# ZechengLi19/CIM

Hardware: AMD Instinct MI355X
Metric: images/sec training step (ResNet-50 VOC, ~1k proposals/img) at 1/2/4/8 GPU (higher is better)
Workload: dtype fp32

## Files before the change

cim_amd/csrc/losses.hip:

```cpp
#include "common.h"
#include "wave_block.h"
#include "../../include/cim_hip.h"
#include <limits.h>

namespace {

constexpr int NT = 1024;
constexpr float LO = 1e-6f, HI = 1.0f - 1e-6f;
#ifndef CIM_LOSS_CLOCKS
#define CIM_LOSS_CLOCKS 0
#endif
#if CIM_LOSS_CLOCKS
__device__ unsigned long long g_loss_clk[8][16];
#define LCLK(JOB, I) do { if (threadIdx.x == 0 && (JOB) < 8) g_loss_clk[JOB][I] = wall_clock64(); } while (0)
#else
#define LCLK(JOB, I) do { } while (0)
#endif

__device__ __forceinline__ float clampf(float x) { return fminf(fmaxf(x, LO), HI); }
__device__ __forceinline__ float inrange(float x) { return (x >= LO && x <= HI) ? 1.0f : 0.0f; }

__device__ float block_sum(float v, float* red) {
#pragma unroll
    for (int o = 32; o > 0; o >>= 1) v += __shfl_xor(v, o);
    const int wave = threadIdx.x >> 6, lane = threadIdx.x & 63;
    __syncthreads();
    if (lane == 0) red[wave] = v;
    __syncthreads();
    float s = 0.0f;
    for (int w = 0; w < NT / 64; ++w) s += red[w];
    return s;
}

__device__ void block_sum4(float& v0, float& v1, float& v2, float& v3, float* buf) {
#pragma unroll
    for (int o = 32; o > 0; o >>= 1) {
// ... 386 lines not shown
                    if (row_cluster[n] != k) continue;
                    const float x = a.pc[(size_t)n * LD + c], p = clampf(x);
                    const float t = (row_col[n] == c) ? 1.0f : 0.0f;
                    s += -(t * logf(p) + (1.0f - t) * logf(1.0f - p));
                    g[(size_t)n * C1 + c] = scale * (-(t / p - (1.0f - t) / (1.0f - p))) / (float)C1 * inrange(x);
                }
    #pragma unroll
                for (int o = 32; o > 0; o >>= 1) s += __shfl_xor(s, o);
                if (lane == 0) acc += s / (float)C1;
            } else {
                float s = 0.0f;
                int any = 0;
                for (int n = lane; n < N; n += 64) {
                    if (row_cluster[n] != k) continue;
                    s += a.pc[(size_t)n * LD + c];
                    any |= (row_col[n] == c);
                }
    #pragma unroll
                for (int o = 32; o > 0; o >>= 1) { s += __shfl_xor(s, o); any |= __shfl_xor(any, o); }
                const float v = s / nk, p = clampf(v), t = any ? 1.0f : 0.0f;
                if (lane == 0) acc += nk * (-(t * logf(p) + (1.0f - t) * logf(1.0f - p))) / (float)C1;
                const float dv = scale * (-(t / p - (1.0f - t) / (1.0f - p))) / (float)C1 * inrange(v);
                for (int n = lane; n < N; n += 64)
                    if (row_cluster[n] == k) g[(size_t)n * C1 + c] = dv;
            }
        }
    }
    LCLK(a.R + 1, 3);
    acc = block_sum(acc, red);
    float* out = a.part + 4 * (a.R + 1);
    if (tid == 0) { out[0] = 0.f; out[1] = scale * acc; out[2] = 0.f; out[3] = 0.f; }
}

__global__ __launch_bounds__(NT) void losses_kernel(const cim_loss_args a) {
    extern __shared__ __attribute__((aligned(16))) unsigned char smem[];
    float* red = reinterpret_cast<float*>(smem);
    int* hot = reinterpret_cast<int*>(smem + 64);
    float* grp_scratch = reinterpret_cast<float*>(smem + 64 + 8 * (size_t)a.N);
    const int job = blockIdx.x;
    LCLK(job, 0);
    if (job < a.R) refine_job(a, job, red, hot, grp_scratch);
    else if (job == a.R) mil_job(a, red, grp_scratch);
    else pcl_job(a, red, smem + 64, grp_scratch);
    LCLK(job, 7);
}

}

#if CIM_LOSS_CLOCKS
extern "C" int cim_debug_loss_clocks(unsigned long long* host_out) {
    return hipMemcpyFromSymbol(host_out, HIP_SYMBOL(g_loss_clk), sizeof(g_loss_clk)) == hipSuccess ? 0 : 1;
}
#endif

extern "C" int cim_losses_fwd(const cim_loss_args* args, void* stream) {
    CIM_CHECK_ARG(args != nullptr);
    const cim_loss_args& a = *args;
    CIM_CHECK_ARG(a.N > 0 && a.N <= 15000 && a.C1 > 1 && a.C1 <= 32767 && a.R >= 0 && a.R <= 3 && (a.ld == 0 || a.ld >= a.C1));
    CIM_CHECK_ARG(a.pc && a.pd && a.labels && a.part && a.grad && a.mat && (a.R == 0 || a.layer_valid));
    for (int i = 0; i < a.R; ++i)
        CIM_CHECK_ARG(a.rc[i] && a.ri[i] && a.pseudo_labels[i] && a.pseudo_iou_f16[i] && a.loss_weights[i]);
    const int lg = a.C1 <= 32 ? 32 : a.C1 <= 64 ? 64 : a.C1 <= 128 ? 128 : a.C1 <= 256 ? 256 : 1024;
    const size_t lds = 64 + 8 * (size_t)a.N + (lg <= 256 ? 16 * (size_t)(NT / lg) * a.C1 + 16 : 0) + 256;
    if (lds > 64 * 1024)
        CIM_CHECK_HIP(hipFuncSetAttribute(reinterpret_cast<const void*>(losses_kernel),
                                          hipFuncAttributeMaxDynamicSharedMemorySize, (int)lds));
    hipLaunchKernelGGL(losses_kernel, dim3(a.R + 2), dim3(NT), lds, cim::as_stream(stream), a);
    CIM_CHECK_LAUNCH();
    return 0;
}

namespace {

__global__ __launch_bounds__(256) void head_colstat_kernel(const float* __restrict__ x, int N, int C1, int ld, int off,
                                                           float* __restrict__ stat) {
    __shared__ float red[4];
    const int c = blockIdx.x, tid = threadIdx.x;
    float m = -INFINITY;
    for (int n = tid; n < N; n += 256) m = fmaxf(m, x[(size_t)n * ld + off + c]);
#pragma unroll
    for (int o = 32; o > 0; o >>= 1) m = fmaxf(m, __shfl_xor(m, o));
    if ((tid & 63) == 0) red[tid >> 6] = m;
    __syncthreads();
    m = fmaxf(fmaxf(red[0], red[1]), fmaxf(red[2], red[3]));
    __syncthreads();
    float s = 0.0f;
    for (int n = tid; n < N; n += 256) s += expf(x[(size_t)n * ld + off + c] - m);
#pragma unroll
    for (int o = 32; o > 0; o >>= 1) s += __shfl_xor(s, o);
    if ((tid & 63) == 0) red[tid >> 6] = s;
    __syncthreads();
    if (tid == 0) {
        stat[c] = m;
        stat[C1 + c] = red[0] + red[1] + red[2] + red[3];
    }
}

__global__ __launch_bounds__(256) void head_act_fwd_kernel(const float* __restrict__ x, float* __restrict__ y, int N, int C1,
                                                           int R, const float* __restrict__ stat) {
    const int row = blockIdx.x * 4 + (threadIdx.x >> 6), lane = threadIdx.x & 63;
    if (row >= N) return;
    const int ld = (2 + 2 * R) * C1;
// ... 27 lines not shown
    for (int n = tid; n < N; n += 256) s += y[(size_t)n * ld + off + c] * dy[(size_t)n * ld + off + c];
#pragma unroll
    for (int o = 32; o > 0; o >>= 1) s += __shfl_xor(s, o);
    if ((tid & 63) == 0) red[tid >> 6] = s;
    __syncthreads();
    if (tid == 0) dot[c] = red[0] + red[1] + red[2] + red[3];
}

__global__ __launch_bounds__(256) void head_act_bwd_kernel(const float* __restrict__ y, const float* __restrict__ dy,
                                                           float* __restrict__ dx, int N, int C1, int R,
                                                           const float* __restrict__ dot) {
    const int row = blockIdx.x * 4 + (threadIdx.x >> 6), lane = threadIdx.x & 63;
    if (row >= N) return;
    const int ld = (2 + 2 * R) * C1;
    const float* yr = y + (size_t)row * ld;
    const float* gr = dy + (size_t)row * ld;
    float* dr = dx + (size_t)row * ld;
    for (int b = 0; b < 2 + 2 * R; ++b) {
        const int off = b * C1;
        if (b == 1) {
            for (int c = lane; c < C1; c += 64) dr[off + c] = yr[off + c] * (gr[off + c] - dot[c]);
        } else if (b < 2 + R) {
            float s = 0.0f;
            for (int c = lane; c < C1; c += 64) s += yr[off + c] * gr[off + c];
#pragma unroll
            for (int o = 32; o > 0; o >>= 1) s += __shfl_xor(s, o);
            for (int c = lane; c < C1; c += 64) dr[off + c] = yr[off + c] * (gr[off + c] - s);
        } else {
            for (int c = lane; c < C1; c += 64) dr[off + c] = gr[off + c] * yr[off + c] * (1.0f - yr[off + c]);
        }
    }
}

struct LossGrads { const float* p[6]; };
__global__ __launch_bounds__(256) void loss_grad_combine_kernel(const float* __restrict__ G, const LossGrads g,
                                                                float* __restrict__ out, int N, int C1, int R) {
    const size_t plane = (size_t)N * C1;
    const size_t i = (size_t)blockIdx.x * 256 + threadIdx.x;
    if (i >= plane) return;
    const int n = (int)(i / C1), c = (int)(i - (size_t)n * C1);
    float v[6];
#pragma unroll
    for (int k = 0; k < 6; ++k) v[k] = g.p[k] ? g.p[k][0] : 0.0f;
    const float g_bag = v[0] + v[5], g_pcl = v[1] + v[5], g_cls = v[2] + v[5], g_iou = v[3] + 3.0f * (v[4] + v[5]);
    float* o = out + (size_t)n * (2 + 2 * R) * C1 + c;
    o[0] = g_bag * G[i] + g_pcl * G[plane + i];
    o[C1] = g_bag * G[2 * plane + i];
    for (int r = 0; r < R; ++r) {
        const float* Gr = G + (size_t)(3 + 4 * r) * plane + i;
        o[(2 + r) * C1] = g_cls * Gr[0] + g_bag * Gr[plane];
        o[(2 + R + r) * C1] = g_iou * Gr[2 * plane] + g_bag * Gr[3 * plane];
    }
}

__global__ void loss_finish_kernel(const float* __restrict__ part, int rows, float* __restrict__ out) {
#pragma clang fp contract(off)
    const int k = threadIdx.x;
    float s = 0.0f;
    if (k < 4)
        for (int r = 0; r < rows; ++r) s += part[r * 4 + k];
    const float bag = __shfl(s, 0), pcl = __shfl(s, 1), cls = __shfl(s, 2), iou = __shfl(s, 3);
    if (k < 4) out[k] = s;
    if (k == 4) out[4] = 3.0f * iou;
    if (k == 5) out[5] = ((bag + pcl) + cls) + 3.0f * iou;
}

}

extern "C" int cim_loss_finish(const float* part, int rows, float* out, void* stream) {
    CIM_CHECK_ARG(part && out && rows > 0);
    hipLaunchKernelGGL(loss_finish_kernel, dim3(1), dim3(64), 0, cim::as_stream(stream), part, rows, out);
    CIM_CHECK_LAUNCH();
    return 0;
}

extern "C" int cim_loss_grad_combine(const float* G, const float* g_bag, const float* g_pcl, const float* g_cls, const float* g_iou,
                                     const float* g_iou3, const float* g_total, float* out, int N, int C1, int R, void* stream) {
    CIM_CHECK_ARG(G && out && N > 0 && C1 > 0 && R >= 0 && R <= 3);
    const LossGrads g{{g_bag, g_pcl, g_cls, g_iou, g_iou3, g_total}};
    const size_t n = (size_t)N * C1;
    hipLaunchKernelGGL(loss_grad_combine_kernel, dim3((unsigned)((n + 255) / 256)), dim3(256), 0, cim::as_stream(stream), G, g, out, N, C1, R);
    CIM_CHECK_LAUNCH();
    return 0;
}

extern "C" int cim_head_act_fwd(const float* logits, float* scores, float* colstat, int N, int C1, int R, void* stream) {
    CIM_CHECK_ARG(logits && scores && colstat && N > 0 && C1 > 0 && R >= 0 && R <= 8);
    const int ld = (2 + 2 * R) * C1;
    hipStream_t st = cim::as_stream(stream);
    hipLaunchKernelGGL(head_colstat_kernel, dim3(C1), dim3(256), 0, st, logits, N, C1, ld, C1, colstat);
    hipLaunchKernelGGL(head_act_fwd_kernel, dim3((N + 3) / 4), dim3(256), 0, st, logits, scores, N, C1, R, colstat);
    CIM_CHECK_LAUNCH();
    return 0;
}

extern "C" int cim_head_act_bwd(const float* scores, const float* grad_scores, float* grad_logits, float* coldot, int N,
                                int C1, int R, void* stream) {
    CIM_CHECK_ARG(scores && grad_scores && grad_logits && coldot && N > 0 && C1 > 0 && R >= 0 && R <= 8);
    const int ld = (2 + 2 * R) * C1;
    hipStream_t st = cim::as_stream(stream);
    hipLaunchKernelGGL(head_coldot_kernel, dim3(C1), dim3(256), 0, st, scores, grad_scores, N, C1, ld, C1, coldot);
    hipLaunchKernelGGL(head_act_bwd_kernel, dim3((N + 3) / 4), dim3(256), 0, st, scores, grad_scores, grad_logits, N, C1, R,
                       coldot);
    CIM_CHECK_LAUNCH();
    return 0;
}
```

cim_amd/modeling/heads.py:

```python
import ctypes
import os
import warnings

import numpy as np
import torch
import torch.nn as nn
import torch.nn.functional as F

from .. import _lib
from ..utils import engine

_EPS = 1e-6


def _clamp(x):
    return x.clamp(_EPS, 1 - _EPS)


def mil_loss(cls_score, labels, loss_weight=None):
    s = _clamp(cls_score)
    t = labels.clamp(0, 1)
    loss = -(t * torch.log(s)) - (1 - t) * torch.log(1 - s)
    if loss_weight is not None:
        loss = loss * loss_weight
    return loss.mean()


def _pad_bg(labels):
    return torch.cat((labels.new_ones(labels.shape[0], 1), labels), dim=1)


def mil_bag_loss(predict_cls, predict_det, labels):
    pred = _clamp((predict_cls * predict_det).sum(dim=0, keepdim=True))
    target = _pad_bg(labels) if pred.shape[-1] - 1 == labels.shape[-1] else labels
    return -(target * torch.log(pred) + (1 - target) * torch.log(1 - pred)).mean()
# ... 60 lines not shown
def PCL_loss(predict_cls, mat, labels):
    ids = torch.unique(mat)
    ids = ids[ids != 0]
    if ids.numel() == 0:
        return 12 * predict_cls.new_zeros(())
    col0 = torch.unique(mat[:, 0])
    col0 = col0[col0 != 0]
    assert col0.numel() <= 1
    eq = mat.unsqueeze(0) == ids.view(-1, 1, 1)
    rows = eq.any(dim=2).to(predict_cls.dtype)
    cols = eq.any(dim=1).to(predict_cls.dtype)
    n_k = rows.sum(dim=1)
    is_bg = (ids == col0[0]) if col0.numel() == 1 else torch.zeros_like(ids, dtype=torch.bool)
    p = _clamp(predict_cls)
    mean_vec = _clamp((rows @ predict_cls) / n_k.clamp(min=1).unsqueeze(1))
    fg_term = (-(cols * torch.log(mean_vec)) - (1 - cols) * torch.log(1 - mean_vec)).mean(dim=1)
    gt = (mat != 0).to(predict_cls.dtype)
    bce_rows = (-(gt * torch.log(p)) - (1 - gt) * torch.log(1 - p)).mean(dim=1)
    bg_term = (rows * bce_rows.unsqueeze(0)).sum(dim=1) / n_k.clamp(min=1)
    term = torch.where(is_bg, bg_term, fg_term) * n_k
    return 12 * (term.sum() / (1e-6 + n_k.sum()))


_LossArgs = _lib.STRUCTS["cim_loss_args"]


STATUS_BITS = {1: "a class produced more than K pseudo ground truths (internal)",
               2: "the pre-drawn uniforms were exhausted (internal)",
               4: "`mat` has rows with several non-zero entries: the fused PCL loss handles the reference's "
                  "one-cluster-per-row format (tools/pre/AGPL_label_assign.py:137-185) - set CIM_PCL_GENERAL=1 for the "
                  "general ATen formulation",
               8: "several distinct cluster ids in column 0 of `mat` (heads.py:20 asserts at most one)",
               16: "more PRM clusters in `mat` than the fused PCL loss supports - set CIM_PCL_GENERAL=1"}


class FusedLossFunction(torch.autograd.Function):

    @staticmethod
    def forward(ctx, meta, pc, pd, *scores):
        R = meta["R"]
        fused = meta.get("fused", False)
        dev = pc.device
        if fused:
            all_scores = pc.contiguous()
            N, C1 = all_scores.shape[0], all_scores.shape[1] // (2 + 2 * R)
            base, blk = all_scores.data_ptr(), 4 * C1
            ptrs = [base + h * blk for h in range(2 + 2 * R)]
            ld = (2 + 2 * R) * C1
        else:
            rc, ri = scores[:R], scores[R:2 * R]
            N, C1 = pc.shape
            pc, pd = pc.contiguous(), pd.contiguous()
            rc = [t.contiguous() for t in rc]
            ri = [t.contiguous() for t in ri]
            ptrs = [pc.data_ptr(), pd.data_ptr()] + [t.data_ptr() for t in rc] + [t.data_ptr() for t in ri]
            ld = 0
        part = torch.empty((R + 2, 4), dtype=torch.float32, device=dev)
        grad = torch.empty((3 + 4 * R, N, C1), dtype=torch.float32, device=dev)
        a = _LossArgs()
        a.pc, a.pd, a.ld = ptrs[0], ptrs[1], ld
        keep = []
        for i in range(R):
            a.rc[i], a.ri[i] = ptrs[2 + i], ptrs[2 + R + i]
            y, t16, w = (x.contiguous() for x in meta["pseudo"][i])
            assert t16.dtype == torch.float16 and y.dtype == torch.float32 and w.dtype == torch.float32
            keep += [y, t16, w]
            a.pseudo_labels[i], a.pseudo_iou_f16[i], a.loss_weights[i] = y.data_ptr(), t16.data_ptr(), w.data_ptr()
            a.weight_scale[i] = float(meta["scales"][i])
        labels = meta["labels"].reshape(-1).to(torch.float32).contiguous()
        mat = meta["mat"].to(torch.float32).contiguous()
        assert tuple(mat.shape) == (N, C1), "mat must be [N, C+1]"
        valid, status = meta["valid"], meta["status"]
        a.labels, a.mat = labels.data_ptr(), mat.data_ptr()
        a.layer_valid, a.status = _lib.ptr(valid), status.data_ptr()
        a.N, a.C1, a.R = N, C1, R
        a.part, a.grad = part.data_ptr(), grad.data_ptr()
        _lib.call("cim_losses_fwd", ctypes.byref(a), _lib.stream_ptr())
        ctx.R, ctx.fused, ctx.dims = R, fused, (N, C1)
        ctx.save_for_backward(grad)
        ctx.set_materialize_grads(False)
        out = torch.empty(6, dtype=torch.float32, device=dev)
        _lib.call("cim_loss_finish", part.data_ptr(), R + 2, out.data_ptr(), _lib.stream_ptr())
        return tuple(out.unbind(0))

    @staticmethod
    def backward(ctx, *g):
        (G,) = ctx.saved_tensors
        R = ctx.R
        if _rng.pending is not None and not LAZY_SETTLE:
            engine.queue_callback(settle_rng)
        _order_callers_stream_after_backward(G.device)
        if ctx.fused:
            N, C1 = ctx.dims
            out = torch.empty((N, (2 + 2 * R) * C1), dtype=torch.float32, device=G.device)
            g = [None if t is None else t.contiguous() for t in g]
            _lib.call("cim_loss_grad_combine", G.data_ptr(), *[_lib.ptr(t) for t in g], out.data_ptr(), N, C1, R, _lib.stream_ptr())
            return None, out, None
        zero = G.new_zeros(())
        v = [zero if t is None else t for t in g]
        g_bag, g_pcl, g_cls, g_iou = v[0] + v[5], v[1] + v[5], v[2] + v[5], v[3] + 3 * (v[4] + v[5])
        d_pc = g_bag * G[0] + g_pcl * G[1]
        d_pd = g_bag * G[2]
        d_rc = [g_cls * G[3 + 4 * i] + g_bag * G[4 + 4 * i] for i in range(R)]
        d_ri = [g_iou * G[5 + 4 * i] + g_bag * G[6 + 4 * i] for i in range(R)]
        return (None, d_pc, d_pd, *d_rc, *d_ri)


def _order_callers_stream_after_backward(dev):
    from ..ops import gemm as _g
    if not (engine.HAS_ENGINE_CALLBACK and _g.HIGH_PRIO and dev.type == "cuda"):
        return

    def order():
        cur = torch.cuda.current_stream(dev)
        hp = _g.main_stream_high_priority(dev)
# ... 22 lines not shown
def fused_losses(predict_cls, predict_det, ref_cls_score, ref_iou_score, labels, pseudo, scales, mat,
                 valid=None, status=None, with_total=False):
    R = len(ref_cls_score)
    dev = predict_cls.device
    pseudo = list(pseudo)
    if valid is None or any(ps is None for ps in pseudo):
        host_valid = torch.tensor([0 if ps is None else 1 for ps in pseudo], dtype=torch.int32)
        valid = host_valid.to(dev) if valid is None else valid * host_valid.to(dev)
        some = next((ps for ps in pseudo if ps is not None), None)
        if some is None:
            n, c1 = predict_cls.shape
            some = (predict_cls.new_zeros((n, c1)), torch.zeros(n, dtype=torch.float16, device=dev), predict_cls.new_zeros(n))
        pseudo = [some if ps is None else ps for ps in pseudo]
    own_status = status is None
    if own_status:
        status = torch.zeros(1, dtype=torch.int32, device=dev)
    meta = dict(R=R, pseudo=pseudo, scales=list(scales), labels=labels, mat=mat, valid=valid, status=status)
    base = _fused_base(predict_cls, predict_det, ref_cls_score, ref_iou_score)
    if base is not None:
        meta["fused"] = True
        out = FusedLossFunction.apply(meta, base, None)
    else:
        out = FusedLossFunction.apply(meta, predict_cls, predict_det, *ref_cls_score, *ref_iou_score)
    if own_status:
        check_status(int(status.item()))
    return tuple(out) if with_total else (out[0], out[1], out[2], out[3])


def check_status(word):
    if word:
        raise _lib.CimHipError("; ".join(msg for bit, msg in STATUS_BITS.items() if word & bit))


class cls_iou_model(nn.Module):

    def __init__(self, dim_in, dim_out, refine_times, class_agnostic=False):
        super().__init__()
        self.classifier = nn.Linear(dim_in, dim_out)
        self.detector = nn.Linear(dim_in, dim_out)
        self.refine_cls = nn.ModuleList([nn.Linear(dim_in, dim_out) for _ in range(refine_times)])
        self.refine_iou = nn.ModuleList([nn.Linear(dim_in, dim_out) for _ in range(refine_times)])

    def detectron_weight_mapping(self):
        return {name: name for name, _ in self.named_parameters()}, []

    def forward(self, seg_feature):
        if seg_feature.dim() == 4:
            seg_feature = seg_feature.squeeze(3).squeeze(2)
        layers = [self.classifier, self.detector] + list(self.refine_cls) + list(self.refine_iou)
        r = len(self.refine_cls)
        c1 = self.classifier.out_features
        if seg_feature.is_cuda and seg_feature.dtype == torch.float32:
            scores = HeadsFunction.apply(seg_feature, c1, r, *[l.weight for l in layers], *[l.bias for l in layers]).split(c1, dim=1)
        else:
            w = torch.cat([l.weight for l in layers], dim=0)
            b = torch.cat([l.bias for l in layers], dim=0)
            logits = F.linear(seg_feature, w, b)
            lg = logits.split(c1, dim=1)
            scores = ([F.softmax(lg[0], dim=-1), F.softmax(lg[1], dim=0)] + [F.softmax(l, dim=-1) for l in lg[2:2 + r]]
                      + [torch.sigmoid(l) for l in lg[2 + r:2 + 2 * r]])
        return scores[0], scores[1], list(scores[2:2 + r]), list(scores[2 + r:2 + 2 * r])


class HeadActFunction(torch.autograd.Function):

    @staticmethod
    def forward(ctx, logits, c1, r):
        logits = logits.contiguous()
        n = logits.shape[0]
        scores = torch.empty_like(logits)
        stat = torch.empty(2 * c1, dtype=torch.float32, device=logits.device)
        _lib.call("cim_head_act_fwd", logits.data_ptr(), scores.data_ptr(), stat.data_ptr(), n, c1, r, _lib.stream_ptr())
        ctx.save_for_backward(scores)
        ctx.dims = (n, c1, r)
        return scores

    @staticmethod
    def backward(ctx, g):
        (scores,) = ctx.saved_tensors
        n, c1, r = ctx.dims
        g = g.contiguous()
        dx = torch.empty_like(scores)
        dot = torch.empty(c1, dtype=torch.float32, device=scores.device)
        _lib.call("cim_head_act_bwd", scores.data_ptr(), g.data_ptr(), dx.data_ptr(), dot.data_ptr(), n, c1, r,
                  _lib.stream_ptr())
        return dx, None, None


def _small_gemm(a, b, c, m, n, k, lda, ldb, ldc, a_mcontig, b_kcontig):
    splits = _lib.call("cim_gemm_small_splits", m, n, k)
    ws = torch.empty(splits * m * n, dtype=torch.float32, device=c.device) if splits > 1 else None
    _lib.call("cim_gemm_small_f32", a.data_ptr(), b.data_ptr(), c.data_ptr(), m, n, k, lda, ldb, ldc, int(a_mcontig), int(b_kcontig),
              None, None, None, None, None, 0.0, None, 0, splits, _lib.ptr(ws), _lib.stream_ptr())


class HeadsFunction(torch.autograd.Function):

    @staticmethod
    def forward(ctx, x, c1, r, *wb):
        nh = 2 + 2 * r
        ws_, bs_ = wb[:nh], wb[nh:]
        x = x.contiguous()
        n, k = x.shape
        wcat = torch.cat([w.detach() for w in ws_], dim=0)
        bcat = torch.cat([b.detach() for b in bs_], dim=0)
        m = nh * c1
        logits = torch.empty((n, m), dtype=torch.float32, device=x.device)
        splits = _lib.call("cim_gemm_small_splits", n, m, k)
        wsp = torch.empty(splits * n * m, dtype=torch.float32, device=x.device) if splits > 1 else None
        _lib.call("cim_linear_bias_f32", x.data_ptr(), wcat.data_ptr(), bcat.data_ptr(), logits.data_ptr(), n, m, k, splits,
                  _lib.ptr(wsp), _lib.stream_ptr())
        scores = torch.empty_like(logits)
        stat = torch.empty(2 * c1, dtype=torch.float32, device=x.device)
        _lib.call("cim_head_act_fwd", logits.data_ptr(), scores.data_ptr(), stat.data_ptr(), n, c1, r, _lib.stream_ptr())
        ctx.save_for_backward(x, wcat, scores)
        ctx.dims = (n, k, c1, r)
        return scores

    @staticmethod
    def backward(ctx, g):
        x, wcat, scores = ctx.saved_tensors
        n, k, c1, r = ctx.dims
        nh = 2 + 2 * r
        m = nh * c1
        g = g.contiguous()
        dl = torch.empty_like(scores)
        dot = torch.empty(c1, dtype=torch.float32, device=scores.device)
        _lib.call("cim_head_act_bwd", scores.data_ptr(), g.data_ptr(), dl.data_ptr(), dot.data_ptr(), n, c1, r, _lib.stream_ptr())
        dx = dw = db = None
        if ctx.needs_input_grad[0]:
            dx = torch.empty((n, k), dtype=torch.float32, device=x.device)
            _small_gemm(dl, wcat, dx, n, k, m, m, k, k, False, False)
        if any(ctx.needs_input_grad[3:3 + nh]):
            dw = torch.empty((m, k), dtype=torch.float32, device=x.device)
            _small_gemm(dl, x, dw, m, k, n, m, k, k, True, False)
        if any(ctx.needs_input_grad[3 + nh:]):
            db = dl.sum(dim=0)
        gw = [dw[h * c1:(h + 1) * c1] if dw is not None and ctx.needs_input_grad[3 + h] else None for h in range(nh)]
        gb = [db[h * c1:(h + 1) * c1] if db is not None and ctx.needs_input_grad[3 + nh + h] else None for h in range(nh)]
        return (dx, None, None, *gw, *gb)


_MiningLayer = _lib.STRUCTS["cim_mining_layer"]
_MiningArgs = _lib.STRUCTS["cim_mining_args"]
MAX_LAYERS = _lib.CONSTANTS["CIM_MAX_LAYERS"]


class _RngLedger:

    def __init__(self):
        self.pending = None
        self.snapshot = None

    def draw(self, n):
        self.settle()
        before = np.random.get_state()
        u = np.random.random_sample(n)
        self.snapshot = (before, np.random.get_state())
        return u

    def commit(self, meta_dev):
        host = torch.empty(meta_dev.numel(), dtype=torch.int32, pin_memory=True)
        host.copy_(meta_dev, non_blocking=True)
        ev = torch.cuda.Event()
        ev.record()
        self.pending = (self.snapshot, host, ev)
        self.snapshot = None
        return host, ev

    def settle(self):
        if self.pending is None:
            return
        snapshot, host, ev = self.pending
# ... 285 lines not shown
```

cim_amd/modeling/model_builder.py:

```python
import importlib
import logging
import os
import pickle
from functools import wraps

import torch
import torch.nn as nn

from ..core.config import cfg
from ..ops import RoIAlign, RoIPool
from ..ops import gemm as _gemm_ops
from . import heads

logger = logging.getLogger(__name__)


def get_func(func_name):
    if func_name == "":
        return None
    try:
        parts = func_name.split(".")
        if len(parts) == 1:
            return globals()[parts[0]]
        module = importlib.import_module(__package__ + "." + ".".join(parts[:-1]))
# ... 81 lines not shown

    def state_dict(self, *args, **kwargs):
        _gemm_ops.wait_pending_updates()
        return super().state_dict(*args, **kwargs)

    def forward(self, data, rois, masks, labels, gtrois=None, mat=None, path=None, index=None,
                iou_map=None, asy_iou_map=None):
        if not (self.training and _gemm_ops.HIGH_PRIO and torch.is_tensor(data) and data.is_cuda) or torch.cuda.is_current_stream_capturing():
            return self._forward_impl(data, rois, masks, labels, gtrois, mat, path, index, iou_map, asy_iou_map)
        dev = data.device
        cur, hp = torch.cuda.current_stream(dev), _gemm_ops.main_stream_high_priority(dev)
        if cur == hp:
            return self._forward_impl(data, rois, masks, labels, gtrois, mat, path, index, iou_map, asy_iou_map)
        hp.wait_stream(cur)
        for t in (data, rois, masks, labels, gtrois, mat, index, iou_map, asy_iou_map):
            if torch.is_tensor(t) and t.is_cuda:
                t.record_stream(hp)
        with torch.cuda.stream(hp):
            out = self._forward_impl(data, rois, masks, labels, gtrois, mat, path, index, iou_map, asy_iou_map)
        cur.wait_stream(hp)
        out["blob_conv"].record_stream(cur)
        for v in out.get("losses", {}).values():
            v.record_stream(cur)
        return out

    def _forward_impl(self, data, rois, masks, labels, gtrois=None, mat=None, path=None, index=None,
                      iou_map=None, asy_iou_map=None):
        with torch.set_grad_enabled(self.training):
            im_data = data
            if self.training:
                _gemm_ops.join_side(discard=True)
                if hasattr(self.Box_Head, "prefetch"):
                    self.Box_Head.prefetch()
                dev, dt = im_data.device, im_data.dtype
                rois = rois.squeeze(dim=0).to(device=dev, dtype=dt)
                masks = masks.squeeze(dim=0).to(device=dev, dtype=dt)
                labels = labels.squeeze(dim=0).to(device=dev, dtype=dt)
                mat = mat.squeeze(dim=0).to(device=dev, dtype=dt)
                if index is not None:
                    index = index.squeeze(dim=0).to(device=dev).long()
            return_dict = {}
            prep = None
            if self.training and asy_iou_map is not None and asy_iou_map.is_cuda:
                prep = heads.prepare_containment(self.CIM_layer_list, asy_iou_map, self.using_CIM)
            blob_conv = self._conv_body(im_data)
            return_dict["blob_conv"] = blob_conv
            seg_x = self.Box_Head(blob_conv, rois, masks.detach())
            predict_cls, predict_det, ref_cls_score, ref_iou_score = self.cls_iou_model(seg_x)

            if not self.training:
                return testing_function(predict_cls, predict_det, ref_cls_score, ref_iou_score, return_dict)

            if iou_map is None or asy_iou_map is None:
                stem = os.path.splitext(os.path.split(path)[1])[0]
                iou_map = _load_map(cfg.iou_dir, stem, "iou_map", labels.device, index)
                asy_iou_map = _load_map(cfg.asy_iou_dir, stem, "asy_iou_map", labels.device, index)

            scores = [(predict_cls, predict_det) if i == 0 else (ref_cls_score[i - 1], ref_iou_score[i - 1])
                      for i in range(len(self.CIM_layer_list))]
            mined = self.__dict__.get("_fixed_mining")
            if mined is None:
                mined = heads.mine_step(self.CIM_layer_list, scores, labels, iou_map, asy_iou_map, self.using_CIM, prep=prep)
            scales = [3 if i == 0 else 1 for i in range(len(self.CIM_layer_list))]
            if cfg.REFINE_TIMES <= 3 and not PCL_GENERAL:
                bag, pcl, cls_l, _, iou3, total = heads.fused_losses(predict_cls, predict_det, ref_cls_score, ref_iou_score,
                                                                     labels, mined.pseudo, scales, mat, valid=mined.valid,
# ... 79 lines not shown
```

cim_amd/nn/parallel/data_parallel.py:

```python
import os
import contextlib

import torch
import torch.distributed as dist

from ...ops.gemm import join_side as _join_side, gradient_is_deferred as _gradient_is_deferred
from ...ops import gemm as _gemm_ops
from ...utils import engine
from torch import nn


class DataParallel(nn.Module):
    def __init__(self, module, device_ids=None, output_device=None, dim=0, cpu_keywords=(), minibatch=False,
                 batch_outputs=True, bucket_bytes=64 << 20, process_group=None, force_flat_grads=False,
                 big_bytes=16 << 20, iter_size=None):
        super().__init__()
        self.module = module
        self.cpu_keywords = list(cpu_keywords)
        self.minibatch = minibatch
        self.batch_outputs = batch_outputs
        self.dim = dim
        self.process_group = process_group
        self.world_size = dist.get_world_size(process_group) if dist.is_available() and dist.is_initialized() else 1
        self.device = next(module.parameters()).device
# ... 69 lines not shown
                close()
        close()
        self._bucket_of = {}
        for bi, bk in enumerate(self.buckets):
            for p in bk["params"]:
                self._bucket_of[p] = bi
        if self.world_size > 1:
            for p in params:
                p.register_post_accumulate_grad_hook(self._on_grad_ready)
            _gemm_ops.register_publisher(params, self._publish_early)
            if not engine.HAS_ENGINE_CALLBACK:
                from torch.optim.optimizer import register_optimizer_step_pre_hook
                self._step_hook = register_optimizer_step_pre_hook(lambda opt, args, kwargs: self._before_optimizer_step())

    def _before_optimizer_step(self):
        self._cb_queued = False
        if self.world_size > 1 and self._sync and not self._reduced_this_step:
            self.finish_gradient_sync()
        self._reduced_this_step = False
        self._fwd_since_step = 0

    def attach_optimizer(self, optimizer, early_modules=("Box_Head", "cls_iou_model")):
        if not hasattr(optimizer, "step_early") or self.device.type != "cuda" or not engine.HAS_ENGINE_CALLBACK:
            return False
        params = []
        for name in early_modules:
            mod = getattr(self.module, name, None)
            if mod is not None:
                params += [p for p in mod.parameters() if p.requires_grad]
        if not params:
            return False
        self._early = (optimizer, params, frozenset(id(p) for p in params), torch.cuda.Stream(device=self.device))
        from ...ops import maskfuse_pair as _mfp
        _mfp.DEFER_DW = False
        if self.world_size == 1:
            for p in params:
                p.register_post_accumulate_grad_hook(self._on_grad_ready)
        return True

    def _maybe_step_early(self, p):
        if self._early is None or id(p) not in self._early[2]:
            return
        self._early_seen += 1
        if self._early_seen < len(self._early[1]) or not self._sync_this_backward():
            return
        opt, params, _, side = self._early
        if self.world_size > 1:
            if any(self._bucket_of[q] >= self._next_bucket for q in params):
                return
            cur = torch.cuda.current_stream()
            side.wait_stream(cur)
            with torch.cuda.stream(side):
                for w, buf in self._pending:
                    w.wait()
                    if buf is not None:
                        buf.div_(self.world_size)
            self._pending = []
        opt.step_early(params, side)

    def _sync_this_backward(self):
        if not engine.HAS_ENGINE_CALLBACK:
            return self._sync and self._fwd_since_step % max(self.iter_size, 1) == 0
        return self._sync and (self._backwards + 1) % max(self.iter_size, 1) == 0

    def _backward_started(self):
        if not self._cb_queued:
            self._cb_queued = True
# ... 146 lines not shown
```

include/cim_hip.h:

```cpp
#ifndef CIM_HIP_H
#define CIM_HIP_H

#include <stdint.h>

#ifdef __cplusplus
extern "C" {
#endif

const char* cim_last_error(void);
int cim_abi_version(void);

int cim_roi_align_fwd(const float* feat, const float* rois, float* out,
                      int B, int C, int H, int W, int K, int P,
                      float spatial_scale, int sampling_ratio, int aligned, void* stream);

long long cim_roi_align_bwd_workspace(int K, int P, int H, int W);
int cim_roi_align_bwd(const float* grad_out, const float* rois, float* grad_in,
                      int B, int C, int H, int W, int K, int P,
                      float spatial_scale, int sampling_ratio, int aligned, float* workspace, void* stream);

int cim_roi_align_fwd_ws(const float* feat, const float* rois, float* out,
                         int B, int C, int H, int W, int K, int P,
                         float spatial_scale, int sampling_ratio, int aligned, float* workspace, void* stream);
int cim_roi_align_maskcat_fwd_ws(const float* feat, const float* rois, const float* masks, float* cat,
// ... 298 lines not shown
int cim_wino7_dx_maskfold(const float* M, const float* masks, float* dbox, int R, int Cb, void* stream);

#define CIM_PCL_MAX_CLUSTERS 256
typedef struct cim_loss_args {
    const float* pc;
    const float* pd;
    const float* rc[3];
    const float* ri[3];
    const float* pseudo_labels[3];
    const uint16_t* pseudo_iou_f16[3];
    const float* loss_weights[3];
    float weight_scale[3];
    const int32_t* layer_valid;
    const float* labels;
    const float* mat;
    int32_t* status;
    int N, C1, R;
    float* part;
    float* grad;
    int ld;
} cim_loss_args;

int cim_losses_fwd(const cim_loss_args* args, void* stream);

int cim_linear_bias_f32(const float* X, const float* W, const float* bias, float* Y, int M, int N, int K, int splits,
                        float* workspace, void* stream);
int cim_loss_finish(const float* part, int rows, float* out, void* stream);
int cim_loss_grad_combine(const float* G, const float* g_bag, const float* g_pcl, const float* g_cls, const float* g_iou,
                          const float* g_iou3, const float* g_total, float* out, int N, int C1, int R, void* stream);
int cim_head_act_fwd(const float* logits, float* scores, float* colstat, int N, int C1, int R, void* stream);
int cim_head_act_bwd(const float* scores, const float* grad_scores, float* grad_logits, float* coldot,
                     int N, int C1, int R, void* stream);

typedef struct cim_sgd_tensor {
    uint64_t p;
    uint64_t g;
    uint64_t buf;
    int64_t n;
    float lr, wd;
    int32_t rows, cols;
    uint64_t row_amax, col_amax;
} cim_sgd_tensor;
typedef struct cim_sgd_chunk {
    int32_t tensor;
    int32_t n;
    int64_t offset;
} cim_sgd_chunk;
int cim_sgd_multi(const cim_sgd_tensor* tensors, const cim_sgd_chunk* chunks, int n_chunks, float momentum, int max_workgroups,
                  void* stream);

typedef struct cim_adam_tensor {
    uint64_t p;
    uint64_t g;
    uint64_t exp_avg;
    uint64_t exp_avg_sq;
    int64_t n;
    float step_size, bc2_sqrt, wd;
    int32_t rows, cols;
    int32_t reserved;
    uint64_t row_amax, col_amax;
} cim_adam_tensor;
int cim_adam_multi(const cim_adam_tensor* tensors, const cim_sgd_chunk* chunks, int n_chunks, double beta1, double beta2, double eps,
                   int max_workgroups, void* stream);

int cim_grad_norm_multi(const uint64_t* grads, const int64_t* numel, int n_tensors,
                        const cim_sgd_chunk* chunks, int n_chunks, double* partial ,
// ... 17 lines not shown
```

Before: 75.64.

## Fuse loss finish into loss kernel, prepack head weights, defer head weight grads

```diff
diff --git a/cim_amd/csrc/losses.hip b/cim_amd/csrc/losses.hip
--- a/cim_amd/csrc/losses.hip
+++ b/cim_amd/csrc/losses.hip
@@ -2,6 +2,8 @@
 #include "wave_block.h"
 #include "../../include/cim_hip.h"
 #include <limits.h>
+#include <algorithm>
+#include <cstdint>
 
 namespace {
 
@@ -454,7 +456,19 @@
     if (tid == 0) { out[0] = 0.f; out[1] = scale * acc; out[2] = 0.f; out[3] = 0.f; }
 }
 
-__global__ __launch_bounds__(NT) void losses_kernel(const cim_loss_args a) {
+template <class Load>
+__device__ __forceinline__ void loss_finish_lanes(Load load, int rows, float* __restrict__ out, int k) {
+#pragma clang fp contract(off)
+    float s = 0.0f;
+    if (k < 4)
+        for (int r = 0; r < rows; ++r) s += load(r * 4 + k);
+    const float bag = __shfl(s, 0), pcl = __shfl(s, 1), cls = __shfl(s, 2), iou = __shfl(s, 3);
+    if (k < 4) out[k] = s;
+    if (k == 4) out[4] = 3.0f * iou;
+    if (k == 5) out[5] = ((bag + pcl) + cls) + 3.0f * iou;
+}
+
+__global__ __launch_bounds__(NT) void losses_kernel(const cim_loss_args a, unsigned* __restrict__ ticket, float* __restrict__ out) {
     extern __shared__ __attribute__((aligned(16))) unsigned char smem[];
     float* red = reinterpret_cast<float*>(smem);
     int* hot = reinterpret_cast<int*>(smem + 64);
@@ -465,6 +479,19 @@
     else if (job == a.R) mil_job(a, red, grp_scratch);
     else pcl_job(a, red, smem + 64, grp_scratch);
     LCLK(job, 7);
+    if (ticket == nullptr) return;
+    __shared__ int s_last;
+    __builtin_amdgcn_fence(__ATOMIC_RELEASE, "agent");
+    __syncthreads();
+    if (threadIdx.x == 0)
+        s_last = __hip_atomic_fetch_add(ticket, 1u, __ATOMIC_ACQ_REL, __HIP_MEMORY_SCOPE_AGENT) == gridDim.x - 1;
+    __syncthreads();
+    if (!s_last || threadIdx.x >= 64) return;
+    __builtin_amdgcn_fence(__ATOMIC_ACQUIRE, "agent");
+    const float* part = a.part;
+    loss_finish_lanes([part](int i) { return __hip_atomic_load(part + i, __ATOMIC_RELAXED, __HIP_MEMORY_SCOPE_AGENT); },
+                      (int)gridDim.x, out, (int)threadIdx.x);
+    if (threadIdx.x == 0) __hip_atomic_store(ticket, 0u, __ATOMIC_RELAXED, __HIP_MEMORY_SCOPE_AGENT);
 }
 
 }
@@ -475,21 +502,38 @@
 }
 #endif
 
-extern "C" int cim_losses_fwd(const cim_loss_args* args, void* stream) {
-    CIM_CHECK_ARG(args != nullptr);
+#define CIM_LOSS_CHECK_ARG(cond)                                                \
+    do {                                                                        \
+        if (!(cond)) {                                                          \
+            cim::set_error("cim_losses_fwd: bad argument: %s", #cond);          \
+            return -1;                                                          \
+        }                                                                       \
+    } while (0)
+
+static int losses_launch(const cim_loss_args* args, unsigned* ticket, float* out, void* stream) {
+    CIM_LOSS_CHECK_ARG(args != nullptr);
     const cim_loss_args& a = *args;
-    CIM_CHECK_ARG(a.N > 0 && a.N <= 15000 && a.C1 > 1 && a.C1 <= 32767 && a.R >= 0 && a.R <= 3 && (a.ld == 0 || a.ld >= a.C1));
-    CIM_CHECK_ARG(a.pc && a.pd && a.labels && a.part && a.grad && a.mat && (a.R == 0 || a.layer_valid));
+    CIM_LOSS_CHECK_ARG(a.N > 0 && a.N <= 15000 && a.C1 > 1 && a.C1 <= 32767 && a.R >= 0 && a.R <= 3 && (a.ld == 0 || a.ld >= a.C1));
+    CIM_LOSS_CHECK_ARG(a.pc && a.pd && a.labels && a.part && a.grad && a.mat && (a.R == 0 || a.layer_valid));
     for (int i = 0; i < a.R; ++i)
-        CIM_CHECK_ARG(a.rc[i] && a.ri[i] && a.pseudo_labels[i] && a.pseudo_iou_f16[i] && a.loss_weights[i]);
+        CIM_LOSS_CHECK_ARG(a.rc[i] && a.ri[i] && a.pseudo_labels[i] && a.pseudo_iou_f16[i] && a.loss_weights[i]);
     const int lg = a.C1 <= 32 ? 32 : a.C1 <= 64 ? 64 : a.C1 <= 128 ? 128 : a.C1 <= 256 ? 256 : 1024;
     const size_t lds = 64 + 8 * (size_t)a.N + (lg <= 256 ? 16 * (size_t)(NT / lg) * a.C1 + 16 : 0) + 256;
     if (lds > 64 * 1024)
         CIM_CHECK_HIP(hipFuncSetAttribute(reinterpret_cast<const void*>(losses_kernel),
                                           hipFuncAttributeMaxDynamicSharedMemorySize, (int)lds));
-    hipLaunchKernelGGL(losses_kernel, dim3(a.R + 2), dim3(NT), lds, cim::as_stream(stream), a);
+    hipLaunchKernelGGL(losses_kernel, dim3(a.R + 2), dim3(NT), lds, cim::as_stream(stream), a, ticket, out);
     CIM_CHECK_LAUNCH();
     return 0;
+}
+
+extern "C" int cim_losses_fwd(const cim_loss_args* args, void* stream) {
+    return losses_launch(args, nullptr, nullptr, stream);
+}
+
+extern "C" int cim_losses_fwd_finish(const cim_loss_args* args, uint32_t* ticket, float* out, void* stream) {
+    CIM_CHECK_ARG(ticket && out);
+    return losses_launch(args, ticket, out, stream);
 }
 
 namespace {
@@ -583,6 +627,26 @@
     }
 }
 
+struct HeadsPack { const float* w[CIM_HEADS_MAX]; const float* b[CIM_HEADS_MAX]; };
+template <bool VEC>
+__global__ __launch_bounds__(256) void heads_pack_kernel(const HeadsPack p, float* __restrict__ wcat, float* __restrict__ bcat,
+                                                         int C1, int K) {
+    const int h = blockIdx.y;
+    const size_t n = (size_t)C1 * K;
+    const float* __restrict__ src = p.w[h];
+    float* __restrict__ dst = wcat + (size_t)h * n;
+    const size_t i0 = (size_t)blockIdx.x * 256 + threadIdx.x, step = (size_t)gridDim.x * 256;
+    if (VEC) {
+        const float4* __restrict__ s4 = reinterpret_cast<const float4*>(src);
+        float4* __restrict__ d4 = reinterpret_cast<float4*>(dst);
+        for (size_t i = i0; i < n / 4; i += step) d4[i] = s4[i];
+    } else {
+        for (size_t i = i0; i < n; i += step) dst[i] = src[i];
+    }
+    if (blockIdx.x == 0)
+        for (int c = threadIdx.x; c < C1; c += 256) bcat[(size_t)h * C1 + c] = p.b[h][c];
+}
+
 struct LossGrads { const float* p[6]; };
 __global__ __launch_bounds__(256) void loss_grad_combine_kernel(const float* __restrict__ G, const LossGrads g,
                                                                 float* __restrict__ out, int N, int C1, int R) {
@@ -605,15 +669,7 @@
 }
 
 __global__ void loss_finish_kernel(const float* __restrict__ part, int rows, float* __restrict__ out) {
-#pragma clang fp contract(off)
-    const int k = threadIdx.x;
-    float s = 0.0f;
-    if (k < 4)
-        for (int r = 0; r < rows; ++r) s += part[r * 4 + k];
-    const float bag = __shfl(s, 0), pcl = __shfl(s, 1), cls = __shfl(s, 2), iou = __shfl(s, 3);
-    if (k < 4) out[k] = s;
-    if (k == 4) out[4] = 3.0f * iou;
-    if (k == 5) out[5] = ((bag + pcl) + cls) + 3.0f * iou;
+    loss_finish_lanes([part](int i) { return part[i]; }, rows, out, (int)threadIdx.x);
 }
 
 }
@@ -656,3 +712,25 @@
     CIM_CHECK_LAUNCH();
     return 0;
 }
+
+extern "C" int cim_heads_pack(const float* const* weights, const float* const* biases, int heads, int C1, int K, float* wcat,
+                              float* bcat, void* stream) {
+    CIM_CHECK_ARG(weights && biases && wcat && bcat && heads > 0 && heads <= CIM_HEADS_MAX && C1 > 0 && K > 0);
+    HeadsPack p{};
+    const size_t n = (size_t)C1 * K;
+    bool vec = n % 4 == 0 && reinterpret_cast<uintptr_t>(wcat) % 16 == 0;
+    for (int h = 0; h < heads; ++h) {
+        CIM_CHECK_ARG(weights[h] && biases[h]);
+        p.w[h] = weights[h];
+        p.b[h] = biases[h];
+        vec = vec && reinterpret_cast<uintptr_t>(weights[h]) % 16 == 0;
+    }
+    const size_t items = vec ? n / 4 : n;
+    const unsigned gx = (unsigned)std::min<size_t>((items + 1023) / 1024, 64);
+    if (vec)
+        hipLaunchKernelGGL(heads_pack_kernel<true>, dim3(gx, heads), dim3(256), 0, cim::as_stream(stream), p, wcat, bcat, C1, K);
+    else
+        hipLaunchKernelGGL(heads_pack_kernel<false>, dim3(gx, heads), dim3(256), 0, cim::as_stream(stream), p, wcat, bcat, C1, K);
+    CIM_CHECK_LAUNCH();
+    return 0;
+}
diff --git a/cim_amd/modeling/heads.py b/cim_amd/modeling/heads.py
--- a/cim_amd/modeling/heads.py
+++ b/cim_amd/modeling/heads.py
@@ -1,6 +1,8 @@
+import contextlib
 import ctypes
 import os
 import warnings
+import weakref
 
 import numpy as np
 import torch
@@ -127,6 +129,17 @@
                   "general ATen formulation",
                8: "several distinct cluster ids in column 0 of `mat` (heads.py:20 asserts at most one)",
                16: "more PRM clusters in `mat` than the fused PCL loss supports - set CIM_PCL_GENERAL=1"}
+
+
+_LOSS_TICKETS = {}
+
+
+def _loss_ticket(dev, stream):
+    key = (dev.index, stream)
+    t = _LOSS_TICKETS.get(key)
+    if t is None and not torch.cuda.is_current_stream_capturing():
+        t = _LOSS_TICKETS[key] = torch.zeros(1, dtype=torch.int32, device=dev)
+    return t
 
 
 class FusedLossFunction(torch.autograd.Function):
@@ -170,12 +183,17 @@
         a.layer_valid, a.status = _lib.ptr(valid), status.data_ptr()
         a.N, a.C1, a.R = N, C1, R
         a.part, a.grad = part.data_ptr(), grad.data_ptr()
-        _lib.call("cim_losses_fwd", ctypes.byref(a), _lib.stream_ptr())
+        out = torch.empty(6, dtype=torch.float32, device=dev)
+        st = _lib.stream_ptr()
+        ticket = _loss_ticket(dev, st)
+        if ticket is not None:
+            _lib.call("cim_losses_fwd_finish", ctypes.byref(a), ticket.data_ptr(), out.data_ptr(), st)
+        else:
+            _lib.call("cim_losses_fwd", ctypes.byref(a), st)
+            _lib.call("cim_loss_finish", part.data_ptr(), R + 2, out.data_ptr(), st)
         ctx.R, ctx.fused, ctx.dims = R, fused, (N, C1)
         ctx.save_for_backward(grad)
         ctx.set_materialize_grads(False)
-        out = torch.empty(6, dtype=torch.float32, device=dev)
-        _lib.call("cim_loss_finish", part.data_ptr(), R + 2, out.data_ptr(), _lib.stream_ptr())
         return tuple(out.unbind(0))
 
     @staticmethod
@@ -264,6 +282,10 @@
         raise _lib.CimHipError("; ".join(msg for bit, msg in STATUS_BITS.items() if word & bit))
 
 
+PREFETCH_PACK = True
+_PACKS = weakref.WeakKeyDictionary()
+
+
 class cls_iou_model(nn.Module):
 
     def __init__(self, dim_in, dim_out, refine_times, class_agnostic=False):
@@ -276,14 +298,67 @@
     def detectron_weight_mapping(self):
         return {name: name for name, _ in self.named_parameters()}, []
 
+    def _layers(self):
+        return [self.classifier, self.detector] + list(self.refine_cls) + list(self.refine_iou)
+
+    def packed(self, ahead=False):
+        from ..ops import gemm as G
+        layers = self._layers()
+        ws, bs = [l.weight for l in layers], [l.bias for l in layers]
+        dev = ws[0].device
+        key = tuple((t._version, t.data_ptr()) for t in ws + bs)
+        e = _PACKS.get(self)
+        if e is not None and e[0] == key:
+            if ahead:
+                return None
+            if e[3] is not None:
+                cur = torch.cuda.current_stream(dev)
+                cur.wait_event(e[3])
+                e[1].record_stream(cur)
+                e[2].record_stream(cur)
+            return e[1], e[2]
+        capturing = torch.cuda.is_current_stream_capturing()
+        if ahead and not (G.OVERLAP and PREFETCH_PACK and ws[0].is_cuda and not capturing and all(t.is_contiguous() for t in ws + bs)):
+            return None
+        if any(t.dtype != torch.float32 or not t.is_cuda for t in ws + bs):
+            raise TypeError("cls_iou_model: the heads' parameters must be float32 CUDA/HIP tensors (no CPU fallback)")
+        nh, (c1, k) = len(layers), ws[0].shape
+        with torch.no_grad():
+            src_w, src_b = [w.detach().contiguous() for w in ws], [b.detach().contiguous() for b in bs]
+            ev = None
+            if ahead:
+                side = G._side_stream(dev)
+                side.wait_stream(torch.cuda.current_stream(dev))
+                where = torch.cuda.stream(side)
+            else:
+                G.wait_pending_updates(dev)
+                where = contextlib.nullcontext()
+            with where:
+                wcat = torch.empty((nh * c1, k), dtype=torch.float32, device=dev)
+                bcat = torch.empty(nh * c1, dtype=torch.float32, device=dev)
+                _lib.call("cim_heads_pack", (ctypes.c_void_p * nh)(*[t.data_ptr() for t in src_w]),
+                          (ctypes.c_void_p * nh)(*[t.data_ptr() for t in src_b]), nh, c1, k, wcat.data_ptr(), bcat.data_ptr(),
+                          _lib.stream_ptr())
+                if ahead:
+                    ev = e[3] if e is not None and e[3] is not None else torch.cuda.Event()
+                    ev.record(side)
+        if not capturing:
+            _PACKS[self] = (key, wcat, bcat, ev)
+        return None if ahead else (wcat, bcat)
+
+    def prefetch(self):
+        if self.classifier.weight.is_cuda:
+            self.packed(ahead=True)
+
     def forward(self, seg_feature):
         if seg_feature.dim() == 4:
             seg_feature = seg_feature.squeeze(3).squeeze(2)
-        layers = [self.classifier, self.detector] + list(self.refine_cls) + list(self.refine_iou)
+        layers = self._layers()
         r = len(self.refine_cls)
         c1 = self.classifier.out_features
         if seg_feature.is_cuda and seg_feature.dtype == torch.float32:
-            scores = HeadsFunction.apply(seg_feature, c1, r, *[l.weight for l in layers], *[l.bias for l in layers]).split(c1, dim=1)
+            scores = HeadsFunction.apply(seg_feature, c1, r, self.packed(), *[l.weight for l in layers],
+                                         *[l.bias for l in layers]).split(c1, dim=1)
         else:
             w = torch.cat([l.weight for l in layers], dim=0)
             b = torch.cat([l.bias for l in layers], dim=0)
@@ -319,24 +394,35 @@
         return dx, None, None
 
 
-def _small_gemm(a, b, c, m, n, k, lda, ldb, ldc, a_mcontig, b_kcontig):
+def _small_gemm(a, b, c, m, n, k, lda, ldb, ldc, a_mcontig, b_kcontig, stream=None):
     splits = _lib.call("cim_gemm_small_splits", m, n, k)
     ws = torch.empty(splits * m * n, dtype=torch.float32, device=c.device) if splits > 1 else None
     _lib.call("cim_gemm_small_f32", a.data_ptr(), b.data_ptr(), c.data_ptr(), m, n, k, lda, ldb, ldc, int(a_mcontig), int(b_kcontig),
-              None, None, None, None, None, 0.0, None, 0, splits, _lib.ptr(ws), _lib.stream_ptr())
+              None, None, None, None, None, 0.0, None, 0, splits, _lib.ptr(ws), _lib.stream_ptr() if stream is None else stream)
+    return ws
+
+
+DEFER_DW = True
 
 
 class HeadsFunction(torch.autograd.Function):
 
     @staticmethod
-    def forward(ctx, x, c1, r, *wb):
+    def forward(ctx, x, c1, r, pack, *wb):
         nh = 2 + 2 * r
         ws_, bs_ = wb[:nh], wb[nh:]
         x = x.contiguous()
         n, k = x.shape
-        wcat = torch.cat([w.detach() for w in ws_], dim=0)
-        bcat = torch.cat([b.detach() for b in bs_], dim=0)
         m = nh * c1
+        if pack is None:
+            wcat = torch.empty((m, k), dtype=torch.float32, device=x.device)
+            bcat = torch.empty(m, dtype=torch.float32, device=x.device)
+            src = [t.detach().contiguous() for t in wb]
+            _lib.call("cim_heads_pack", (ctypes.c_void_p * nh)(*[t.data_ptr() for t in src[:nh]]),
+                      (ctypes.c_void_p * nh)(*[t.data_ptr() for t in src[nh:]]), nh, c1, k, wcat.data_ptr(), bcat.data_ptr(),
+                      _lib.stream_ptr())
+        else:
+            wcat, bcat = pack
         logits = torch.empty((n, m), dtype=torch.float32, device=x.device)
         splits = _lib.call("cim_gemm_small_splits", n, m, k)
         wsp = torch.empty(splits * n * m, dtype=torch.float32, device=x.device) if splits > 1 else None
@@ -347,30 +433,54 @@
         _lib.call("cim_head_act_fwd", logits.data_ptr(), scores.data_ptr(), stat.data_ptr(), n, c1, r, _lib.stream_ptr())
         ctx.save_for_backward(x, wcat, scores)
         ctx.dims = (n, k, c1, r)
+        ctx.params = wb
         return scores
 
     @staticmethod
     def backward(ctx, g):
+        from ..ops import chain, gemm as G
         x, wcat, scores = ctx.saved_tensors
         n, k, c1, r = ctx.dims
         nh = 2 + 2 * r
         m = nh * c1
+        dev = x.device
+        need = ctx.needs_input_grad
+        need_w, need_b = any(need[4:4 + nh]), any(need[4 + nh:])
+        st = _lib.stream_ptr()
         g = g.contiguous()
         dl = torch.empty_like(scores)
-        dot = torch.empty(c1, dtype=torch.float32, device=scores.device)
-        _lib.call("cim_head_act_bwd", scores.data_ptr(), g.data_ptr(), dl.data_ptr(), dot.data_ptr(), n, c1, r, _lib.stream_ptr())
-        dx = dw = db = None
-        if ctx.needs_input_grad[0]:
-            dx = torch.empty((n, k), dtype=torch.float32, device=x.device)
+        dot = torch.empty(c1, dtype=torch.float32, device=dev)
+        _lib.call("cim_head_act_bwd", scores.data_ptr(), g.data_ptr(), dl.data_ptr(), dot.data_ptr(), n, c1, r, st)
+        wanted = [q for q, nd in zip(ctx.params, need[4:]) if nd]
+        defer = (DEFER_DW and G.DEFER_DW and bool(wanted) and not torch.cuda.is_current_stream_capturing()
+                 and all(isinstance(q, torch.nn.Parameter) and q.is_leaf and G.publisher_for(q) is None for q in wanted)
+                 and not chain.restricted_pass(ctx, range(len(ctx.next_functions))))
+        side = None
+        if defer:
+            side = G._body_stream(dev)
+            side.wait_stream(torch.cuda.current_stream(dev))
+            st = side.cuda_stream
+        dx = dw = db = ws = None
+        if need[0]:
+            dx = torch.empty((n, k), dtype=torch.float32, device=dev)
             _small_gemm(dl, wcat, dx, n, k, m, m, k, k, False, False)
-        if any(ctx.needs_input_grad[3:3 + nh]):
-            dw = torch.empty((m, k), dtype=torch.float32, device=x.device)
-            _small_gemm(dl, x, dw, m, k, n, m, k, k, True, False)
-        if any(ctx.needs_input_grad[3 + nh:]):
-            db = dl.sum(dim=0)
-        gw = [dw[h * c1:(h + 1) * c1] if dw is not None and ctx.needs_input_grad[3 + h] else None for h in range(nh)]
-        gb = [db[h * c1:(h + 1) * c1] if db is not None and ctx.needs_input_grad[3 + nh + h] else None for h in range(nh)]
-        return (dx, None, None, *gw, *gb)
+        if need_w:
+            dw = torch.empty((m, k), dtype=torch.float32, device=dev)
+            ws = _small_gemm(dl, x, dw, m, k, n, m, k, k, True, False, stream=st)
+        if need_b:
+            db = torch.empty(m, dtype=torch.float32, device=dev)
+            with (torch.cuda.stream(side) if defer else contextlib.nullcontext()):
+                torch.sum(dl, dim=0, out=db)
+        gw = [dw[h * c1:(h + 1) * c1] if dw is not None and need[4 + h] else None for h in range(nh)]
+        gb = [db[h * c1:(h + 1) * c1] if db is not None and need[4 + nh + h] else None for h in range(nh)]
+        if defer:
+            keep = [t for t in (dl, x, ws, dw, db) if t is not None]
+            for q, t in zip(ctx.params, gw + gb):
+                if t is not None:
+                    G.defer_side_join(dev, q, t, *keep)
+                    keep = []
+            return (dx, None, None, None) + (None,) * (2 * nh)
+        return (dx, None, None, None, *gw, *gb)
 
 
 _MiningLayer = _lib.STRUCTS["cim_mining_layer"]
diff --git a/cim_amd/modeling/model_builder.py b/cim_amd/modeling/model_builder.py
--- a/cim_amd/modeling/model_builder.py
+++ b/cim_amd/modeling/model_builder.py
@@ -137,6 +137,8 @@
                 _gemm_ops.join_side(discard=True)
                 if hasattr(self.Box_Head, "prefetch"):
                     self.Box_Head.prefetch()
+                if hasattr(self.cls_iou_model, "prefetch"):
+                    self.cls_iou_model.prefetch()
                 dev, dt = im_data.device, im_data.dtype
                 rois = rois.squeeze(dim=0).to(device=dev, dtype=dt)
                 masks = masks.squeeze(dim=0).to(device=dev, dtype=dt)
diff --git a/cim_amd/nn/parallel/data_parallel.py b/cim_amd/nn/parallel/data_parallel.py
--- a/cim_amd/nn/parallel/data_parallel.py
+++ b/cim_amd/nn/parallel/data_parallel.py
@@ -125,7 +125,9 @@
             return False
         self._early = (optimizer, params, frozenset(id(p) for p in params), torch.cuda.Stream(device=self.device))
         from ...ops import maskfuse_pair as _mfp
+        from ...modeling import heads as _heads
         _mfp.DEFER_DW = False
+        _heads.DEFER_DW = False
         if self.world_size == 1:
             for p in params:
                 p.register_post_accumulate_grad_hook(self._on_grad_ready)
diff --git a/include/cim_hip.h b/include/cim_hip.h
--- a/include/cim_hip.h
+++ b/include/cim_hip.h
@@ -354,6 +354,11 @@
 int cim_head_act_bwd(const float* scores, const float* grad_scores, float* grad_logits, float* coldot,
                      int N, int C1, int R, void* stream);
 
+#define CIM_HEADS_MAX 18
+int cim_losses_fwd_finish(const cim_loss_args* args, uint32_t* ticket, float* out, void* stream);
+int cim_heads_pack(const float* const* weights, const float* const* biases, int heads, int C1, int K, float* wcat, float* bcat,
+                   void* stream);
+
 typedef struct cim_sgd_tensor {
     uint64_t p;
     uint64_t g;
```

Result: no change. 76.26, median of 6 (+0.8%).
